# ZackHodari/morgana

Measured on AMD Instinct MI355X. Metric: acoustic frames/sec (fwd+bwd+step), F0Model 600->1, batch 256x1000, higher is better.
Workload: dtype bf16

## Files before the change

### morgana_amd/csrc/optim.hip

```cpp
#include "common.h"
#include "expand_reduce.h"

#include <math.h>

struct mg_adam_out {
    float p, m, v;
};
__device__ __forceinline__ mg_adam_out mg_adam_update(float p, float g, float mi, float vi, float beta1, float beta2, float eps,
                                                       float weight_decay, float step_size, float bc2_sqrt, float grad_scale) {
#pragma clang fp contract(off)
    g = g * grad_scale;
    if (weight_decay != 0.f) g = __fmaf_rn(weight_decay, p, g);
    mi = __fmaf_rn(g - mi, 1.f - beta1, mi);
    vi = __fmaf_rn((1.f - beta2) * g, g, vi * beta2);
    const float denom = sqrtf(vi) / bc2_sqrt + eps;
    p = p - step_size * (mi / denom);
    return mg_adam_out{p, mi, vi};
}

__global__ __launch_bounds__(256) void adam_kernel(float* __restrict__ param, const float* __restrict__ grad,
                                                   float* __restrict__ m, float* __restrict__ v, int64_t n, float beta1,
                                                   float beta2, float eps, float weight_decay, float step_size,
                                                   float bc2_sqrt, float grad_scale) {
    for (int64_t i = (int64_t)blockIdx.x * 256 + threadIdx.x; i < n; i += (int64_t)gridDim.x * 256) {
        const mg_adam_out o = mg_adam_update(param[i], grad[i], m[i], v[i], beta1, beta2, eps, weight_decay, step_size, bc2_sqrt, grad_scale);
        param[i] = o.p;
        m[i] = o.m;
        v[i] = o.v;
    }
}

__global__ __launch_bounds__(256) void adam_dev_kernel(float* __restrict__ param, const float* __restrict__ grad,
                                                       float* __restrict__ m, float* __restrict__ v, int64_t n, float beta1,
                                                       float beta2, float eps, float weight_decay,
                                                       const float* __restrict__ scalars, float grad_scale) {
    const float step_size = scalars[0], bc2_sqrt = scalars[1];
    for (int64_t i = (int64_t)blockIdx.x * 256 + threadIdx.x; i < n; i += (int64_t)gridDim.x * 256) {
        const mg_adam_out o = mg_adam_update(param[i], grad[i], m[i], v[i], beta1, beta2, eps, weight_decay, step_size, bc2_sqrt, grad_scale);
        param[i] = o.p;
        m[i] = o.m;
        v[i] = o.v;
    }
}

__global__ __launch_bounds__(256) void adam_plan_kernel(float* __restrict__ param, float* __restrict__ grad, float* __restrict__ m,
                                                        float* __restrict__ v, int64_t n, float beta1, float beta2, float eps,
                                                        float weight_decay, const float* __restrict__ scalars, float grad_scale,
                                                        mg_adam_plan plan, int wide_chunks) {
    __shared__ float part[16][68];
    if (plan.tail.frames > 0 || plan.tail.n > 0) {
        const mg_adam_tail& t = plan.tail;
        const int64_t by_frames = (t.frames + 2047) / 2048;
        int riders = (int)(by_frames > 1 ? by_frames : 1);
        if (riders > (int)gridDim.x) riders = (int)gridDim.x;
        if ((int)blockIdx.x < riders) {
            const int64_t chunks = (t.n + 15) / 16;
            const ExpandReduceArgs xr{t.table, t.rows, t.frames, t.out, t.partial, t.n_partial, t.slab, t.n, t.stride, t.n_slabs, t.dst,
                                      t.n > 0 ? (t.n - 1) / 16 : chunks};
            mg_expand_reduce_rider<256>(xr, (int)blockIdx.x, riders, reinterpret_cast<unsigned char*>(part));
        }
    }
    const float step_size = scalars[0], bc2_sqrt = scalars[1];
    auto update = [&](int64_t i, float g) {
        if (plan.clear_grad) grad[i] = 0.f;
        const mg_adam_out o = mg_adam_update(param[i], g, m[i], v[i], beta1, beta2, eps, weight_decay, step_size, bc2_sqrt, grad_scale);
        const float w = o.p;
        param[i] = w;
        m[i] = o.m;
        v[i] = o.v;
        for (int k = 0; k < plan.n_shadows; ++k) {
            const mg_adam_shadow sh = plan.shadows[k];
            const int64_t j = i - sh.offset;
            if (j < 0 || j >= (int64_t)sh.rows * sh.cols) continue;
            const unsigned r = (unsigned)j / (unsigned)sh.cols, cc = (unsigned)j - r * (unsigned)sh.cols;
            const uint16_t b = mg_f2bf(w);
            if (sh.dst) sh.dst[(size_t)r * sh.ldd + cc] = b;
            if (sh.dst_t) sh.dst_t[(size_t)cc * sh.ldt + r] = b;
            if (sh.pair) {
                const uint16_t lo = mg_f2bf(w - mg_bf2f(b));
                if (sh.dst) sh.dst[(size_t)r * sh.ldd + (sh.ldd >> 1) + cc] = lo;
                if (sh.dst_t) sh.dst_t[(size_t)cc * sh.ldt + (sh.ldt >> 1) + r] = lo;
            }
        }
    };
    const int e = threadIdx.x & 15, p = threadIdx.x >> 4;
    auto slab_chunk = [&](int64_t base) {
        const int64_t i0 = base + 4 * e;
        f32x4 acc = {0.f, 0.f, 0.f, 0.f};
        bool any = false;
        for (int k = 0; k < plan.n_slab_srcs; ++k) {
            const mg_adam_slab_src src = plan.slabs[k];
            const int64_t j0 = i0 - src.begin;
            if (j0 + 3 < 0 || j0 >= src.count) continue;
            any = true;
            if (j0 >= 0 && j0 + 3 < src.count && ((j0 | src.stride) & 3) == 0 && ((uintptr_t)src.slab & 15) == 0) {
                for (int s = p; s < src.n_slabs; s += 16) acc += *reinterpret_cast<const f32x4*>(src.slab + (size_t)s * src.stride + j0);
            } else {
#pragma unroll
                for (int c = 0; c < 4; ++c) {
                    const int64_t j = j0 + c;
                    if (j < 0 || j >= src.count) continue;
                    float t = 0.f;
                    for (int s = p; s < src.n_slabs; s += 16) t += src.slab[(size_t)s * src.stride + j];
                    acc[c] += t;
                }
            }
        }
        const bool block_any = __syncthreads_or(any ? 1 : 0) != 0;
        if (block_any) {
            *reinterpret_cast<f32x4*>(&part[p][4 * e]) = acc;
            __syncthreads();
        }
        if (threadIdx.x < 64) {
            const int64_t i = base + threadIdx.x;
            if (i < n) {
                float g = grad[i];
                if (block_any) {
#pragma unroll
                    for (int q = 0; q < 16; ++q) g += part[q][threadIdx.x];
                }
                update(i, g);
            }
        }
        if (block_any) __syncthreads();
    };
    if (wide_chunks) {
        const int64_t n_chunks = (n + 255) / 256;
        for (int64_t c = n_chunks - 1 - (int64_t)blockIdx.x; c >= 0; c -= (int64_t)gridDim.x) {
            const int64_t sbase = c * 256;
            bool hit = false;
            for (int k = 0; k < plan.n_slab_srcs; ++k)
                if (sbase < plan.slabs[k].begin + plan.slabs[k].count && sbase + 256 > plan.slabs[k].begin) hit = true;
            if (!hit) {
                const int64_t i = sbase + threadIdx.x;
                if (i < n) update(i, grad[i]);
                continue;
            }
            for (int sub = 3; sub >= 0; --sub)
                if (sbase + 64 * sub < n) slab_chunk(sbase + 64 * sub);
        }
        return;
    }
    const int64_t n_chunks = (n + 63) / 64;
    for (int64_t c = n_chunks - 1 - (int64_t)blockIdx.x; c >= 0; c -= (int64_t)gridDim.x) slab_chunk(c * 64);
}

__global__ __launch_bounds__(256) void ema_kernel(float* __restrict__ shadow, const float* __restrict__ param, int64_t n, float one_minus_decay) {
    for (int64_t i = (int64_t)blockIdx.x * 256 + threadIdx.x; i < n; i += (int64_t)gridDim.x * 256) {
        const float s = shadow[i];
        shadow[i] = s - one_minus_decay * (s - param[i]);
    }
}

__global__ __launch_bounds__(256) void cast_pad_bf16_kernel(const float* __restrict__ src, int lds, uint16_t* __restrict__ dst,
                                                            int ldd, int64_t rows, int cols) {
    const int64_t n = rows * ldd;
    for (int64_t i = (int64_t)blockIdx.x * 256 + threadIdx.x; i < n; i += (int64_t)gridDim.x * 256) {
        const int64_t r = i / ldd;
        const int c = (int)(i - r * ldd);
        dst[i] = c < cols ? mg_f2bf(src[r * lds + c]) : (uint16_t)0;
    }
}

__global__ __launch_bounds__(256) void cast_pad_bf16_x8_kernel(const float* __restrict__ src, int lds, uint16_t* __restrict__ dst,
                                                               int ldd, int64_t rows, int cols) {
    const int chunks = ldd >> 3;
    const int64_t n = rows * chunks;
    for (int64_t i = (int64_t)blockIdx.x * 256 + threadIdx.x; i < n; i += (int64_t)gridDim.x * 256) {
        const int64_t r = i / chunks;
        const int c0 = (int)(i - r * chunks) << 3;
        float v[8];
        const float* sp = src + r * lds + c0;
        if (c0 + 8 <= cols) {
            const f32x4 a = *reinterpret_cast<const f32x4*>(sp), b = *reinterpret_cast<const f32x4*>(sp + 4);
            v[0] = a.x; v[1] = a.y; v[2] = a.z; v[3] = a.w;
            v[4] = b.x; v[5] = b.y; v[6] = b.z; v[7] = b.w;
        } else {
#pragma unroll
            for (int j = 0; j < 8; ++j) v[j] = (c0 + j < cols) ? sp[j] : 0.f;
        }
        bf16x8 o;
#pragma unroll
        for (int j = 0; j < 8; ++j) o[j] = (short)mg_f2bf(v[j]);
        *reinterpret_cast<bf16x8*>(dst + r * ldd + c0) = o;
    }
}

__global__ __launch_bounds__(256) void cast_transpose_bf16_kernel(const float* __restrict__ src, int lds, uint16_t* __restrict__ dst,
                                                                  int ldd, int rows, int cols) {
    __shared__ float tile[32][33];
    const int r0 = blockIdx.y * 32, c0 = blockIdx.x * 32;
    const int tx = threadIdx.x & 31, ty = threadIdx.x >> 5;
    for (int j = ty; j < 32; j += 8) {
        const int r = r0 + j, c = c0 + tx;
        tile[j][tx] = (r < rows && c < cols) ? src[(size_t)r * lds + c] : 0.f;
    }
    __syncthreads();
    for (int j = ty; j < 32; j += 8) {
        const int c = c0 + j, r = r0 + tx;
        if (c < cols && r < ldd) dst[(size_t)c * ldd + r] = r < rows ? mg_f2bf(tile[tx][j]) : (uint16_t)0;
    }
}

__global__ __launch_bounds__(256) void cast_bf16_f32_kernel(const uint16_t* __restrict__ src, int lds, float* __restrict__ dst,
                                                            int ldd, int64_t rows, int cols) {
    const int64_t n = rows * cols;
    for (int64_t i = (int64_t)blockIdx.x * 256 + threadIdx.x; i < n; i += (int64_t)gridDim.x * 256) {
        const int64_t r = i / cols;
        const int c = (int)(i - r * cols);
        dst[r * ldd + c] = mg_bf2f(src[r * lds + c]);
    }
}

__global__ __launch_bounds__(256) void sigmoid_kernel(const float* __restrict__ x, float* __restrict__ y, int64_t n) {
    for (int64_t i = (int64_t)blockIdx.x * 256 + threadIdx.x; i < n; i += (int64_t)gridDim.x * 256) y[i] = mg_sigmoid(x[i]);
}

__global__ __launch_bounds__(256) void sigmoid_grad_kernel(const float* __restrict__ dy, const float* __restrict__ y,
                                                           float* __restrict__ dx, int64_t n) {
    for (int64_t i = (int64_t)blockIdx.x * 256 + threadIdx.x; i < n; i += (int64_t)gridDim.x * 256) {
        const float s = y[i];
        dx[i] = dy[i] * s * (1.f - s);
    }
}

template <int ACT>
__global__ __launch_bounds__(256) void act_kernel(const float* __restrict__ x, float* __restrict__ y, int64_t n) {
    for (int64_t i = (int64_t)blockIdx.x * 256 + threadIdx.x; i < n; i += (int64_t)gridDim.x * 256) {
        const float v = x[i];
        y[i] = ACT == MG_ACT_SIGMOID ? mg_sigmoid(v) : ACT == MG_ACT_TANH ? tanhf(v) : mg_relu(v);
    }
}

template <int EPI>
__global__ __launch_bounds__(256) void act_grad_kernel(const float* __restrict__ dy, const float* __restrict__ y, float* __restrict__ dx,
                                                       int64_t n) {
    for (int64_t i = (int64_t)blockIdx.x * 256 + threadIdx.x; i < n; i += (int64_t)gridDim.x * 256) dx[i] = mg_epi_dact<EPI>(dy[i], y[i]);
}

struct CastBatch {
    int count;
    mg_cast_desc d[MG_CAST_MAX];
};

__global__ __launch_bounds__(256) void cast_params_kernel(CastBatch batch) {
    __shared__ float tile[32][33];
    const mg_cast_desc d = batch.d[blockIdx.y];
    if (d.dst) {
        const int64_t n = (int64_t)d.rows * d.ldd;
        for (int64_t i = (int64_t)blockIdx.x * 256 + threadIdx.x; i < n; i += (int64_t)gridDim.x * 256) {
            const int r = (int)(i / d.ldd), c = (int)(i - (int64_t)r * d.ldd);
            d.dst[i] = c < d.cols ? mg_f2bf(d.src[(size_t)r * d.cols + c]) : (uint16_t)0;
        }
    }
    if (d.dst_t) {
        const int tiles_c = (d.cols + 31) / 32, tiles_r = (d.ldt + 31) / 32;
        const int tx = threadIdx.x & 31, ty = threadIdx.x >> 5;
        for (int t = blockIdx.x; t < tiles_c * tiles_r; t += gridDim.x) {
            const int c0 = (t % tiles_c) * 32, r0 = (t / tiles_c) * 32;
            __syncthreads();
            for (int j = ty; j < 32; j += 8) {
                const int r = r0 + j, c = c0 + tx;
                tile[j][tx] = (r < d.rows && c < d.cols) ? d.src[(size_t)r * d.cols + c] : 0.f;
            }
            __syncthreads();
            for (int j = ty; j < 32; j += 8) {
                const int c = c0 + j, r = r0 + tx;
                if (c < d.cols && r < d.ldt) d.dst_t[(size_t)c * d.ldt + r] = r < d.rows ? mg_f2bf(tile[tx][j]) : (uint16_t)0;
            }
        }
    }
}

struct CopyBatch {
    mg_copy_desc d[MG_COPY_MAX];
};

__global__ __launch_bounds__(256) void copy_many_kernel(CopyBatch batch) {
    const mg_copy_desc d = batch.d[blockIdx.y];
    const unsigned char* src = reinterpret_cast<const unsigned char*>(d.src);
    unsigned char* dst = reinterpret_cast<unsigned char*>(d.dst);
    const int64_t stride = (int64_t)gridDim.x * 256;
    if ((((uintptr_t)src | (uintptr_t)dst) & 15) == 0) {
        const int64_t n16 = d.bytes >> 4;
        typedef unsigned int cm_u32x4 __attribute__((ext_vector_type(4)));
        for (int64_t i = (int64_t)blockIdx.x * 256 + threadIdx.x; i < n16; i += stride)
            reinterpret_cast<cm_u32x4*>(dst)[i] = reinterpret_cast<const cm_u32x4*>(src)[i];
        for (int64_t i = (n16 << 4) + (int64_t)blockIdx.x * 256 + threadIdx.x; i < d.bytes; i += stride) dst[i] = src[i];
    } else {
        for (int64_t i = (int64_t)blockIdx.x * 256 + threadIdx.x; i < d.bytes; i += stride) dst[i] = src[i];
    }
}

static int flat_grid(int64_t n) {
    int64_t blocks = mg_ceil_div(n, 256 * 4);
    if (blocks > 4096) blocks = 4096;
    return (int)(blocks < 1 ? 1 : blocks);
}

extern "C" {

int mg_adam_step_f32(float* param, const float* grad, float* exp_avg, float* exp_avg_sq, int64_t n, float lr, float beta1,
                     float beta2, float eps, float weight_decay, int64_t step, float grad_scale, void* stream) {
    MG_CHECK_ARG(param && grad && exp_avg && exp_avg_sq && n >= 0 && step >= 1, "mg_adam_step_f32: bad arguments (n=%lld step=%lld)",
                 (long long)n, (long long)step);
    if (n == 0) return MG_OK;
    const double bc1 = 1.0 - pow((double)beta1, (double)step);
    const double bc2 = 1.0 - pow((double)beta2, (double)step);
    const float step_size = (float)((double)lr / bc1);
    const float bc2_sqrt = (float)sqrt(bc2);
    hipLaunchKernelGGL(adam_kernel, dim3(flat_grid(n)), dim3(256), 0, (hipStream_t)stream, param, grad, exp_avg, exp_avg_sq, n,
                       beta1, beta2, eps, weight_decay, step_size, bc2_sqrt, grad_scale);
    MG_CHECK_LAUNCH("mg_adam_step_f32");
    return MG_OK;
}

__global__ void store_pair_kernel(float* __restrict__ dst, float a, float b) {
    dst[0] = a;
    dst[1] = b;
}

int mg_store_pair_f32(float* dst, float a, float b, void* stream) {
    MG_CHECK_ARG(dst, "mg_store_pair_f32: null destination");
    hipLaunchKernelGGL(store_pair_kernel, dim3(1), dim3(1), 0, (hipStream_t)stream, dst, a, b);
    MG_CHECK_LAUNCH("mg_store_pair_f32");
    return MG_OK;
}

struct StorePairs {
    float v[2 * MG_STORE_PAIRS_MAX];
};
__global__ void store_pairs_kernel(float* __restrict__ dst, StorePairs values, int n) {
    if ((int)threadIdx.x < 2 * n) dst[threadIdx.x] = values.v[threadIdx.x];
}

int mg_store_pairs_f32(float* dst, const float* values, int n_pairs, void* stream) {
    MG_CHECK_ARG(dst && values && n_pairs >= 1 && n_pairs <= MG_STORE_PAIRS_MAX, "mg_store_pairs_f32: bad arguments (n_pairs=%d, at most %d)", n_pairs,
                 MG_STORE_PAIRS_MAX);
    StorePairs sp;
    for (int i = 0; i < 2 * n_pairs; ++i) sp.v[i] = values[i];
    for (int i = 2 * n_pairs; i < 2 * MG_STORE_PAIRS_MAX; ++i) sp.v[i] = 0.f;
    hipLaunchKernelGGL(store_pairs_kernel, dim3(1), dim3(64), 0, (hipStream_t)stream, dst, sp, n_pairs);
    MG_CHECK_LAUNCH("mg_store_pairs_f32");
    return MG_OK;
}

void mg_adam_scalars(float lr, float beta1, float beta2, int64_t step, float* out2) {
    const double bc1 = 1.0 - pow((double)beta1, (double)step);
    const double bc2 = 1.0 - pow((double)beta2, (double)step);
    out2[0] = (float)((double)lr / bc1);
    out2[1] = (float)sqrt(bc2);
}

int mg_adam_step_dev_f32(float* param, const float* grad, float* exp_avg, float* exp_avg_sq, int64_t n, float beta1, float beta2,
                         float eps, float weight_decay, const float* scalars, float grad_scale, void* stream) {
    MG_CHECK_ARG(param && grad && exp_avg && exp_avg_sq && scalars && n >= 0, "mg_adam_step_dev_f32: bad arguments (n=%lld)", (long long)n);
    if (n == 0) return MG_OK;
    hipLaunchKernelGGL(adam_dev_kernel, dim3(flat_grid(n)), dim3(256), 0, (hipStream_t)stream, param, grad, exp_avg, exp_avg_sq, n,
                       beta1, beta2, eps, weight_decay, scalars, grad_scale);
    MG_CHECK_LAUNCH("mg_adam_step_dev_f32");
    return MG_OK;
}

int mg_adam_step_plan_f32(float* param, float* grad, float* exp_avg, float* exp_avg_sq, int64_t n, float beta1, float beta2, float eps,
                          float weight_decay, const float* scalars, float grad_scale, const mg_adam_plan* plan, void* stream) {
    MG_CHECK_ARG(param && grad && exp_avg && exp_avg_sq && scalars && plan && n >= 0, "mg_adam_step_plan_f32: bad arguments (n=%lld)", (long long)n);
    MG_CHECK_ARG(plan->n_slab_srcs >= 0 && plan->n_slab_srcs <= MG_ADAM_MAX_SLABS && plan->n_shadows >= 0 && plan->n_shadows <= MG_ADAM_MAX_SHADOWS,
                 "mg_adam_step_plan_f32: %d slab sources / %d shadows exceed %d / %d", plan->n_slab_srcs, plan->n_shadows, MG_ADAM_MAX_SLABS,
                 MG_ADAM_MAX_SHADOWS);
    for (int k = 0; k < plan->n_slab_srcs; ++k) {
        const mg_adam_slab_src& src = plan->slabs[k];
        MG_CHECK_ARG(src.slab && src.begin >= 0 && src.count > 0 && src.begin + src.count <= n && src.n_slabs >= 1 && src.stride >= src.count,
                     "mg_adam_step_plan_f32: slab source %d (begin %lld count %lld of %lld, %d slabs, stride %lld)", k, (long long)src.begin,
                     (long long)src.count, (long long)n, src.n_slabs, (long long)src.stride);
    }
    for (int k = 0; k < plan->n_shadows; ++k) {
        const mg_adam_shadow& sh = plan->shadows[k];
        MG_CHECK_ARG(sh.offset >= 0 && sh.rows > 0 && sh.cols > 0 && (int64_t)sh.rows * sh.cols < 2147483647LL &&
                         sh.offset + (int64_t)sh.rows * sh.cols <= n && (sh.dst || sh.dst_t),
                     "mg_adam_step_plan_f32: shadow %d does not lie inside the flat buffer", k);
        MG_CHECK_ARG((!sh.dst || sh.ldd >= sh.cols) && (!sh.dst_t || sh.ldt >= sh.rows), "mg_adam_step_plan_f32: shadow %d: ldd %d / ldt %d too small", k,
                     sh.ldd, sh.ldt);
        MG_CHECK_ARG(!sh.pair || ((!sh.dst || (sh.ldd % 2 == 0 && sh.ldd / 2 >= sh.cols)) && (!sh.dst_t || (sh.ldt % 2 == 0 && sh.ldt / 2 >= sh.rows))),
                     "mg_adam_step_plan_f32: shadow %d: pair planes need even ldd %d / ldt %d with half of it covering the matrix", k, sh.ldd, sh.ldt);
    }
    {
        const mg_adam_tail& t = plan->tail;
        MG_CHECK_ARG(t.frames >= 0 && t.n >= 0 && (t.frames == 0 || (t.table && t.rows && t.out)) &&
                         (t.n == 0 || (t.slab && t.dst && t.stride >= t.n && t.n_slabs >= 1 && (t.n_partial == 0 || t.partial))),
                     "mg_adam_step_plan_f32: bad deferred tail (frames %lld, n %lld)", (long long)t.frames, (long long)t.n);
        MG_CHECK_ARG((t.frames == 0 && t.n == 0) || n > 0, "mg_adam_step_plan_f32: a deferred tail needs a launch (n = 0)");
    }
    if (n == 0) return MG_OK;
    int64_t covered = 0;
    for (int k = 0; k < plan->n_slab_srcs; ++k) covered += plan->slabs[k].count;
    const int wide = 2 * covered < n ? 1 : 0;
    hipLaunchKernelGGL(adam_plan_kernel, dim3((unsigned)mg_ceil_div(n, wide ? 256 : 64)), dim3(256), 0, (hipStream_t)stream, param, grad, exp_avg,
                       exp_avg_sq, n, beta1, beta2, eps, weight_decay, scalars, grad_scale, *plan, wide);
    MG_CHECK_LAUNCH("mg_adam_step_plan_f32");
    return MG_OK;
}

int mg_ema_update_f32(float* shadow, const float* param, int64_t n, float decay, void* stream) {
    MG_CHECK_ARG(shadow && param && n >= 0, "mg_ema_update_f32: bad arguments");
    if (n == 0) return MG_OK;
    hipLaunchKernelGGL(ema_kernel, dim3(flat_grid(n)), dim3(256), 0, (hipStream_t)stream, shadow, param, n, 1.0f - decay);
    MG_CHECK_LAUNCH("mg_ema_update_f32");
    return MG_OK;
}

int mg_cast_pad_bf16(const float* src, int lds, uint16_t* dst, int ldd, int64_t rows, int cols, void* stream) {
    MG_CHECK_ARG(src && dst && rows >= 0 && cols > 0 && lds >= cols && ldd >= cols, "mg_cast_pad_bf16: bad arguments (rows=%lld cols=%d lds=%d ldd=%d)",
                 (long long)rows, cols, lds, ldd);
    if (rows == 0) return MG_OK;
    if (lds % 4 == 0 && ldd % 8 == 0 && (((uintptr_t)src | (uintptr_t)dst) % 16) == 0)
        hipLaunchKernelGGL(cast_pad_bf16_x8_kernel, dim3(flat_grid(rows * (ldd / 8))), dim3(256), 0, (hipStream_t)stream, src, lds, dst, ldd, rows, cols);
    else
        hipLaunchKernelGGL(cast_pad_bf16_kernel, dim3(flat_grid(rows * ldd)), dim3(256), 0, (hipStream_t)stream, src, lds, dst, ldd, rows, cols);
    MG_CHECK_LAUNCH("mg_cast_pad_bf16");
    return MG_OK;
}

int mg_cast_transpose_bf16(const float* src, int lds, uint16_t* dst, int ldd, int rows, int cols, void* stream) {
    MG_CHECK_ARG(src && dst && rows > 0 && cols > 0 && lds >= cols && ldd >= rows, "mg_cast_transpose_bf16: bad arguments (rows=%d cols=%d lds=%d ldd=%d)",
                 rows, cols, lds, ldd);
    dim3 grid((unsigned)mg_ceil_div(cols, 32), (unsigned)mg_ceil_div(ldd, 32));
    hipLaunchKernelGGL(cast_transpose_bf16_kernel, grid, dim3(256), 0, (hipStream_t)stream, src, lds, dst, ldd, rows, cols);
    MG_CHECK_LAUNCH("mg_cast_transpose_bf16");
    return MG_OK;
}

int mg_cast_params_bf16(const mg_cast_desc* descs, int count, void* stream) {
    MG_CHECK_ARG(descs && count > 0 && count <= MG_CAST_MAX, "mg_cast_params_bf16: count %d not in 1..%d", count, MG_CAST_MAX);
    CastBatch batch;
    batch.count = count;
    for (int i = 0; i < count; ++i) {
        const mg_cast_desc& d = descs[i];
        MG_CHECK_ARG(d.src && d.rows > 0 && d.cols > 0 && (d.dst || d.dst_t), "mg_cast_params_bf16: bad descriptor %d", i);
        MG_CHECK_ARG(!d.dst || d.ldd >= d.cols, "mg_cast_params_bf16: descriptor %d: ldd %d < cols %d", i, d.ldd, d.cols);
        MG_CHECK_ARG(!d.dst_t || d.ldt >= d.rows, "mg_cast_params_bf16: descriptor %d: ldt %d < rows %d", i, d.ldt, d.rows);
        batch.d[i] = d;
    }
    hipLaunchKernelGGL(cast_params_kernel, dim3(256, count), dim3(256), 0, (hipStream_t)stream, batch);
    MG_CHECK_LAUNCH("mg_cast_params_bf16");
    return MG_OK;
}

int mg_copy_many(const mg_copy_desc* descs, int count, void* stream) {
    MG_CHECK_ARG(descs && count > 0 && count <= MG_COPY_MAX, "mg_copy_many: count %d not in 1..%d", count, MG_COPY_MAX);
    CopyBatch batch;
    int64_t most = 0;
    for (int i = 0; i < count; ++i) {
        MG_CHECK_ARG(descs[i].bytes >= 0 && (descs[i].bytes == 0 || (descs[i].src && descs[i].dst)), "mg_copy_many: bad descriptor %d", i);
        batch.d[i] = descs[i];
        if (descs[i].bytes > most) most = descs[i].bytes;
    }
    if (most == 0) return MG_OK;
    int64_t blocks = mg_ceil_div(most, 256 * 16 * 4);
    if (blocks > 2048) blocks = 2048;
    if (blocks < 1) blocks = 1;
    hipLaunchKernelGGL(copy_many_kernel, dim3((unsigned)blocks, count), dim3(256), 0, (hipStream_t)stream, batch);
    MG_CHECK_LAUNCH("mg_copy_many");
    return MG_OK;
}

int mg_cast_bf16_f32(const uint16_t* src, int lds, float* dst, int ldd, int64_t rows, int cols, void* stream) {
    MG_CHECK_ARG(src && dst && rows >= 0 && cols > 0 && lds >= cols && ldd >= cols, "mg_cast_bf16_f32: bad arguments");
    if (rows == 0) return MG_OK;
    hipLaunchKernelGGL(cast_bf16_f32_kernel, dim3(flat_grid(rows * cols)), dim3(256), 0, (hipStream_t)stream, src, lds, dst, ldd, rows, cols);
    MG_CHECK_LAUNCH("mg_cast_bf16_f32");
    return MG_OK;
}

int mg_sigmoid_f32(const float* x, float* y, int64_t n, void* stream) {
    MG_CHECK_ARG(x && y && n >= 0, "mg_sigmoid_f32: bad arguments");
    if (n == 0) return MG_OK;
    hipLaunchKernelGGL(sigmoid_kernel, dim3(flat_grid(n)), dim3(256), 0, (hipStream_t)stream, x, y, n);
    MG_CHECK_LAUNCH("mg_sigmoid_f32");
    return MG_OK;
}

int mg_sigmoid_grad_f32(const float* dy, const float* y, float* dx, int64_t n, void* stream) {
    MG_CHECK_ARG(dy && y && dx && n >= 0, "mg_sigmoid_grad_f32: bad arguments");
    if (n == 0) return MG_OK;
    hipLaunchKernelGGL(sigmoid_grad_kernel, dim3(flat_grid(n)), dim3(256), 0, (hipStream_t)stream, dy, y, dx, n);
    MG_CHECK_LAUNCH("mg_sigmoid_grad_f32");
    return MG_OK;
}

int mg_act_f32(const float* x, float* y, int64_t n, int act, void* stream) {
    MG_CHECK_ARG(x && y && n >= 0, "mg_act_f32: bad arguments");
    MG_CHECK_ARG(act == MG_ACT_SIGMOID || act == MG_ACT_TANH || act == MG_ACT_RELU, "mg_act_f32: unknown activation %d", act);
    if (n == 0) return MG_OK;
    if (act == MG_ACT_SIGMOID) hipLaunchKernelGGL(act_kernel<MG_ACT_SIGMOID>, dim3(flat_grid(n)), dim3(256), 0, (hipStream_t)stream, x, y, n);
    else if (act == MG_ACT_TANH) hipLaunchKernelGGL(act_kernel<MG_ACT_TANH>, dim3(flat_grid(n)), dim3(256), 0, (hipStream_t)stream, x, y, n);
    else hipLaunchKernelGGL(act_kernel<MG_ACT_RELU>, dim3(flat_grid(n)), dim3(256), 0, (hipStream_t)stream, x, y, n);
    MG_CHECK_LAUNCH("mg_act_f32");
    return MG_OK;
}

int mg_act_grad_f32(const float* dy, const float* y, float* dx, int64_t n, int act, void* stream) {
    MG_CHECK_ARG(dy && y && dx && n >= 0, "mg_act_grad_f32: bad arguments");
    MG_CHECK_ARG(act == MG_ACT_SIGMOID || act == MG_ACT_TANH || act == MG_ACT_RELU, "mg_act_grad_f32: unknown activation %d", act);
    if (n == 0) return MG_OK;
#define ACT_GRAD(EPI_) hipLaunchKernelGGL(act_grad_kernel<EPI_>, dim3(flat_grid(n)), dim3(256), 0, (hipStream_t)stream, dy, y, dx, n)
    MG_SWITCH_GRAD_EPI(mg_epi_grad(act), ACT_GRAD);
#undef ACT_GRAD
    MG_CHECK_LAUNCH("mg_act_grad_f32");
    return MG_OK;
}

}
```

### morgana_amd/csrc/slab_reduce.h

```cpp
#pragma once

#include "common.h"

static __global__ __launch_bounds__(256) void mg_slab_reduce_kernel(const float* __restrict__ slab, int64_t n, int64_t stride,
                                                                    int S, float* __restrict__ dst, int accumulate) {
    __shared__ float part[16][17];
    const int e = threadIdx.x & 15, p = threadIdx.x >> 4;
    for (int64_t base = (int64_t)blockIdx.x * 16; base < n; base += (int64_t)gridDim.x * 16) {
        const int64_t i = base + e;
        float v = 0.f;
        if (i < n) {
#pragma unroll 4
            for (int s = p; s < S; s += 16) v += slab[(size_t)s * stride + i];
        }
        part[p][e] = v;
        __syncthreads();
        if (p == 0 && i < n) {
            float t = accumulate ? dst[i] : 0.f;
#pragma unroll
            for (int q = 0; q < 16; ++q) t += part[q][e];
            dst[i] = t;
        }
        __syncthreads();
    }
}

static __global__ __launch_bounds__(256) void mg_slab_reduce4_kernel(const float* __restrict__ slab, int64_t n, int64_t stride,
                                                                     int S, float* __restrict__ dst, int accumulate) {
    __shared__ f32x4 part[16][17];
    const int e = threadIdx.x & 15, p = threadIdx.x >> 4;
    for (int64_t base = (int64_t)blockIdx.x * 64; base < n; base += (int64_t)gridDim.x * 64) {
        const int64_t i = base + 4 * e;
        f32x4 v = {0.f, 0.f, 0.f, 0.f};
        if (i < n) {
#pragma unroll 4
            for (int s = p; s < S; s += 16) v += *reinterpret_cast<const f32x4*>(slab + (size_t)s * stride + i);
        }
        part[p][e] = v;
        __syncthreads();
        if (p == 0 && i < n) {
            f32x4 t = {0.f, 0.f, 0.f, 0.f};
            if (accumulate) t = *reinterpret_cast<const f32x4*>(dst + i);
#pragma unroll
            for (int q = 0; q < 16; ++q) t += part[q][e];
            *reinterpret_cast<f32x4*>(dst + i) = t;
        }
        __syncthreads();
    }
}

static inline void mg_launch_slab_reduce(const float* slab, int64_t n, int64_t stride, int S, float* dst, int accumulate,
                                         hipStream_t st) {
#ifdef MG_EXPERIMENTS
    if (g_mg_tuning[MG_TUNE_SKIP_REDUCE]) return;
#endif
    if (n % 4 == 0 && stride % 4 == 0 && n >= 4096 && (((uintptr_t)slab | (uintptr_t)dst) % 16) == 0) {
        int64_t blocks4 = mg_ceil_div(n, 64);
        if (blocks4 > 32768) blocks4 = 32768;
        hipLaunchKernelGGL(mg_slab_reduce4_kernel, dim3((unsigned)blocks4), dim3(256), 0, st, slab, n, stride, S, dst, accumulate);
        return;
    }
    int64_t blocks = mg_ceil_div(n, 16);
    if (blocks > 32768) blocks = 32768;
    if (blocks < 1) blocks = 1;
    hipLaunchKernelGGL(mg_slab_reduce_kernel, dim3((unsigned)blocks), dim3(256), 0, st, slab, n, stride, S, dst, accumulate);
}
```

Baseline: 2.499 billion.

## Restructure fused Adam kernel to per-wave 256-element chunks with register slab sums

The fused Adam plan kernel is rewritten so that each wave owns a 256-element chunk, with lanes processing four elements through vectorised loads and stores. The cross-thread reduction through shared memory and its block barriers is replaced by per-lane register accumulation of slab partial sums, with loads batched 16 or 32 at a time. The grid is capped at a fixed block count with launch bounds asking for two blocks per CU, and bf16 shadow writes are packed four at a time. The risks are high register pressure from the 16 f32x4 accumulators, and much less parallelism across the slab dimension, since each lane now serially sums all slabs.

```diff
diff --git a/morgana_amd/csrc/optim.hip b/morgana_amd/csrc/optim.hip
--- a/morgana_amd/csrc/optim.hip
+++ b/morgana_amd/csrc/optim.hip
@@ -1,5 +1,6 @@
 #include "common.h"
 #include "expand_reduce.h"
+#include "slab_reduce.h"
 
 #include <math.h>
 
@@ -43,12 +44,23 @@
     }
 }
 
-__global__ __launch_bounds__(256) void adam_plan_kernel(float* __restrict__ param, float* __restrict__ grad, float* __restrict__ m,
-                                                        float* __restrict__ v, int64_t n, float beta1, float beta2, float eps,
-                                                        float weight_decay, const float* __restrict__ scalars, float grad_scale,
-                                                        mg_adam_plan plan, int wide_chunks) {
-    __shared__ float part[16][68];
+__device__ __noinline__ void mg_adam_edge_sums(const float* __restrict__ slab, int64_t stride, int S, int64_t j0, int64_t count, float* t) {
+    for (int e = 0; e < 4; ++e) {
+        const int64_t j = j0 + e;
+        if (j < 0 || j >= count) continue;
+        for (int s = 0; s < S; ++s) t[(s & 15) * 4 + e] += slab[(int64_t)s * stride + j];
+    }
+}
+
+#ifndef MG_ADAM_PLAN_BLOCKS
+#define MG_ADAM_PLAN_BLOCKS 1024
+#endif
+__global__ __launch_bounds__(256, 2) void adam_plan_kernel(float* __restrict__ param, float* __restrict__ grad, float* __restrict__ m,
+                                                           float* __restrict__ v, int64_t n, float beta1, float beta2, float eps,
+                                                           float weight_decay, const float* __restrict__ scalars, float grad_scale,
+                                                           mg_adam_plan plan) {
     if (plan.tail.frames > 0 || plan.tail.n > 0) {
+        __shared__ float rider_scratch[16 * 17 + 256];
         const mg_adam_tail& t = plan.tail;
         const int64_t by_frames = (t.frames + 2047) / 2048;
         int riders = (int)(by_frames > 1 ? by_frames : 1);
@@ -57,92 +69,144 @@
             const int64_t chunks = (t.n + 15) / 16;
             const ExpandReduceArgs xr{t.table, t.rows, t.frames, t.out, t.partial, t.n_partial, t.slab, t.n, t.stride, t.n_slabs, t.dst,
                                       t.n > 0 ? (t.n - 1) / 16 : chunks};
-            mg_expand_reduce_rider<256>(xr, (int)blockIdx.x, riders, reinterpret_cast<unsigned char*>(part));
+            mg_expand_reduce_rider<256>(xr, (int)blockIdx.x, riders, reinterpret_cast<unsigned char*>(rider_scratch));
         }
     }
     const float step_size = scalars[0], bc2_sqrt = scalars[1];
-    auto update = [&](int64_t i, float g) {
-        if (plan.clear_grad) grad[i] = 0.f;
-        const mg_adam_out o = mg_adam_update(param[i], g, m[i], v[i], beta1, beta2, eps, weight_decay, step_size, bc2_sqrt, grad_scale);
-        const float w = o.p;
-        param[i] = w;
-        m[i] = o.m;
-        v[i] = o.v;
+    auto put = [&](const mg_adam_shadow& sh, unsigned r, unsigned cc, float w, bool hi_done) {
+        const uint16_t b = mg_f2bf(w);
+        if (sh.dst && !hi_done) sh.dst[(size_t)r * sh.ldd + cc] = b;
+        if (sh.dst_t) sh.dst_t[(size_t)cc * sh.ldt + r] = b;
+        if (sh.pair) {
+            const uint16_t lo = mg_f2bf(w - mg_bf2f(b));
+            if (sh.dst) sh.dst[(size_t)r * sh.ldd + (sh.ldd >> 1) + cc] = lo;
+            if (sh.dst_t) sh.dst_t[(size_t)cc * sh.ldt + (sh.ldt >> 1) + r] = lo;
+        }
+    };
+    const int lane = threadIdx.x & 63;
+    const unsigned voff = 16u * (unsigned)lane;
+    const int wave = __builtin_amdgcn_readfirstlane((int)(threadIdx.x >> 6));
+    const bool state_vec = ((((uintptr_t)param | (uintptr_t)grad | (uintptr_t)m | (uintptr_t)v) & 15) == 0);
+    const int64_t n_chunks = (n + 255) / 256;
+    for (int64_t c = n_chunks - 1 - ((int64_t)wave * gridDim.x + blockIdx.x); c >= 0; c -= 4 * (int64_t)gridDim.x) {
+        const int64_t base = c * 256, i0 = base + 4 * lane;
+        const bool whole = state_vec && base + 256 <= n;
+        f32x4 g4 = {0.f, 0.f, 0.f, 0.f}, p4 = g4, m4 = g4, v4 = g4;
+        if (whole) {
+            g4 = *reinterpret_cast<const f32x4*>(grad + i0);
+            p4 = *reinterpret_cast<const f32x4*>(param + i0);
+            m4 = *reinterpret_cast<const f32x4*>(m + i0);
+            v4 = *reinterpret_cast<const f32x4*>(v + i0);
+        } else {
+#pragma unroll
+            for (int e = 0; e < 4; ++e)
+                if (i0 + e < n) {
+                    g4[e] = grad[i0 + e];
+                    p4[e] = param[i0 + e];
+                    m4[e] = m[i0 + e];
+                    v4[e] = v[i0 + e];
+                }
+        }
+        f32x4 t[16];
+#pragma unroll
+        for (int q = 0; q < 16; ++q) t[q] = f32x4{0.f, 0.f, 0.f, 0.f};
+        unsigned covered = 0;
+#pragma unroll 1
+        for (int k = 0; k < plan.n_slab_srcs; ++k) {
+            const mg_adam_slab_src src = plan.slabs[k];
+            const int64_t jb = base - src.begin;
+            if (jb + 256 <= 0 || jb >= src.count) continue;
+            const int64_t j0 = jb + 4 * lane;
+#pragma unroll
+            for (int e = 0; e < 4; ++e)
+                if (j0 + e >= 0 && j0 + e < src.count) covered |= 1u << e;
+            if (((jb | src.stride) & 3) == 0 && ((uintptr_t)src.slab & 15) == 0) {
+                const bool inside = j0 >= 0 && j0 < src.count;
+                const float* sp = src.slab + jb;
+                mg_slab_partition_sums(src.n_slabs, t, [&](int s) {
+                    f32x4 x = {0.f, 0.f, 0.f, 0.f};
+                    if (inside) x = *reinterpret_cast<const f32x4*>(reinterpret_cast<const char*>(sp + (size_t)s * src.stride) + voff);
+                    return x;
+                });
+            } else {
+                float tm[64];
+#pragma unroll
+                for (int q = 0; q < 16; ++q)
+#pragma unroll
+                    for (int e = 0; e < 4; ++e) tm[4 * q + e] = t[q][e];
+                mg_adam_edge_sums(src.slab, src.stride, src.n_slabs, j0, src.count, tm);
+#pragma unroll
+                for (int q = 0; q < 16; ++q)
+#pragma unroll
+                    for (int e = 0; e < 4; ++e) t[q][e] = tm[4 * q + e];
+            }
+        }
+        if (covered) {
+            f32x4 gs = g4;
+#pragma unroll
+            for (int q = 0; q < 16; ++q) gs += t[q];
+#pragma unroll
+            for (int e = 0; e < 4; ++e)
+                if (covered >> e & 1) g4[e] = gs[e];
+        }
+        f32x4 w4;
+#pragma unroll
+        for (int e = 0; e < 4; ++e) {
+            const mg_adam_out o = mg_adam_update(p4[e], g4[e], m4[e], v4[e], beta1, beta2, eps, weight_decay, step_size, bc2_sqrt, grad_scale);
+            w4[e] = o.p;
+            m4[e] = o.m;
+            v4[e] = o.v;
+        }
+        if (whole) {
+            if (plan.clear_grad) *reinterpret_cast<f32x4*>(grad + i0) = f32x4{0.f, 0.f, 0.f, 0.f};
+            *reinterpret_cast<f32x4*>(param + i0) = w4;
+            *reinterpret_cast<f32x4*>(m + i0) = m4;
+            *reinterpret_cast<f32x4*>(v + i0) = v4;
+        } else {
+#pragma unroll
+            for (int e = 0; e < 4; ++e)
+                if (i0 + e < n) {
+                    if (plan.clear_grad) grad[i0 + e] = 0.f;
+                    param[i0 + e] = w4[e];
+                    m[i0 + e] = m4[e];
+                    v[i0 + e] = v4[e];
+                }
+        }
+#pragma unroll 1
         for (int k = 0; k < plan.n_shadows; ++k) {
             const mg_adam_shadow sh = plan.shadows[k];
-            const int64_t j = i - sh.offset;
-            if (j < 0 || j >= (int64_t)sh.rows * sh.cols) continue;
-            const unsigned r = (unsigned)j / (unsigned)sh.cols, cc = (unsigned)j - r * (unsigned)sh.cols;
-            const uint16_t b = mg_f2bf(w);
-            if (sh.dst) sh.dst[(size_t)r * sh.ldd + cc] = b;
-            if (sh.dst_t) sh.dst_t[(size_t)cc * sh.ldt + r] = b;
-            if (sh.pair) {
-                const uint16_t lo = mg_f2bf(w - mg_bf2f(b));
-                if (sh.dst) sh.dst[(size_t)r * sh.ldd + (sh.ldd >> 1) + cc] = lo;
-                if (sh.dst_t) sh.dst_t[(size_t)cc * sh.ldt + (sh.ldt >> 1) + r] = lo;
-            }
-        }
-    };
-    const int e = threadIdx.x & 15, p = threadIdx.x >> 4;
-    auto slab_chunk = [&](int64_t base) {
-        const int64_t i0 = base + 4 * e;
-        f32x4 acc = {0.f, 0.f, 0.f, 0.f};
-        bool any = false;
-        for (int k = 0; k < plan.n_slab_srcs; ++k) {
-            const mg_adam_slab_src src = plan.slabs[k];
-            const int64_t j0 = i0 - src.begin;
-            if (j0 + 3 < 0 || j0 >= src.count) continue;
-            any = true;
-            if (j0 >= 0 && j0 + 3 < src.count && ((j0 | src.stride) & 3) == 0 && ((uintptr_t)src.slab & 15) == 0) {
-                for (int s = p; s < src.n_slabs; s += 16) acc += *reinterpret_cast<const f32x4*>(src.slab + (size_t)s * src.stride + j0);
+            const int64_t rc = (int64_t)sh.rows * sh.cols, jb = base - sh.offset;
+            if (jb + 256 <= 0 || jb >= rc) continue;
+            const int64_t j0 = jb + 4 * lane;
+            if (j0 + 3 < 0 || j0 >= rc) continue;
+            const unsigned jf = (unsigned)(j0 > 0 ? j0 : 0), cols = (unsigned)sh.cols;
+            unsigned r = jf / cols, cc = jf - r * cols;
+            if (j0 >= 0 && j0 + 3 < rc && cc + 3 < cols) {
+                uint16_t* d = sh.dst ? sh.dst + (size_t)r * sh.ldd + cc : nullptr;
+                const bool packed = d && ((uintptr_t)d & 7) == 0;
+                if (packed) {
+                    bf16x4 b;
+#pragma unroll
+                    for (int e = 0; e < 4; ++e) b[e] = (short)mg_f2bf(w4[e]);
+                    *reinterpret_cast<bf16x4*>(d) = b;
+                }
+                if (!packed || sh.dst_t || sh.pair) {
+#pragma unroll
+                    for (int e = 0; e < 4; ++e) put(sh, r, cc + e, w4[e], packed);
+                }
             } else {
 #pragma unroll
-                for (int c = 0; c < 4; ++c) {
-                    const int64_t j = j0 + c;
-                    if (j < 0 || j >= src.count) continue;
-                    float t = 0.f;
-                    for (int s = p; s < src.n_slabs; s += 16) t += src.slab[(size_t)s * src.stride + j];
-                    acc[c] += t;
+                for (int e = 0; e < 4; ++e) {
+                    if (j0 + e < 0 || j0 + e >= rc) continue;
+                    put(sh, r, cc, w4[e], false);
+                    if (++cc == cols) {
+                        cc = 0;
+                        ++r;
+                    }
                 }
             }
         }
-        const bool block_any = __syncthreads_or(any ? 1 : 0) != 0;
-        if (block_any) {
-            *reinterpret_cast<f32x4*>(&part[p][4 * e]) = acc;
-            __syncthreads();
-        }
-        if (threadIdx.x < 64) {
-            const int64_t i = base + threadIdx.x;
-            if (i < n) {
-                float g = grad[i];
-                if (block_any) {
-#pragma unroll
-                    for (int q = 0; q < 16; ++q) g += part[q][threadIdx.x];
-                }
-                update(i, g);
-            }
-        }
-        if (block_any) __syncthreads();
-    };
-    if (wide_chunks) {
-        const int64_t n_chunks = (n + 255) / 256;
-        for (int64_t c = n_chunks - 1 - (int64_t)blockIdx.x; c >= 0; c -= (int64_t)gridDim.x) {
-            const int64_t sbase = c * 256;
-            bool hit = false;
-            for (int k = 0; k < plan.n_slab_srcs; ++k)
-                if (sbase < plan.slabs[k].begin + plan.slabs[k].count && sbase + 256 > plan.slabs[k].begin) hit = true;
-            if (!hit) {
-                const int64_t i = sbase + threadIdx.x;
-                if (i < n) update(i, grad[i]);
-                continue;
-            }
-            for (int sub = 3; sub >= 0; --sub)
-                if (sbase + 64 * sub < n) slab_chunk(sbase + 64 * sub);
-        }
-        return;
-    }
-    const int64_t n_chunks = (n + 63) / 64;
-    for (int64_t c = n_chunks - 1 - (int64_t)blockIdx.x; c >= 0; c -= (int64_t)gridDim.x) slab_chunk(c * 64);
+    }
 }
 
 __global__ __launch_bounds__(256) void ema_kernel(float* __restrict__ shadow, const float* __restrict__ param, int64_t n, float one_minus_decay) {
@@ -392,11 +456,10 @@
         MG_CHECK_ARG((t.frames == 0 && t.n == 0) || n > 0, "mg_adam_step_plan_f32: a deferred tail needs a launch (n = 0)");
     }
     if (n == 0) return MG_OK;
-    int64_t covered = 0;
-    for (int k = 0; k < plan->n_slab_srcs; ++k) covered += plan->slabs[k].count;
-    const int wide = 2 * covered < n ? 1 : 0;
-    hipLaunchKernelGGL(adam_plan_kernel, dim3((unsigned)mg_ceil_div(n, wide ? 256 : 64)), dim3(256), 0, (hipStream_t)stream, param, grad, exp_avg,
-                       exp_avg_sq, n, beta1, beta2, eps, weight_decay, scalars, grad_scale, *plan, wide);
+    int64_t blocks = mg_ceil_div(n, 256);
+    if (blocks > MG_ADAM_PLAN_BLOCKS) blocks = MG_ADAM_PLAN_BLOCKS;
+    hipLaunchKernelGGL(adam_plan_kernel, dim3((unsigned)blocks), dim3(256), 0, (hipStream_t)stream, param, grad, exp_avg, exp_avg_sq, n, beta1,
+                       beta2, eps, weight_decay, scalars, grad_scale, *plan);
     MG_CHECK_LAUNCH("mg_adam_step_plan_f32");
     return MG_OK;
 }
diff --git a/morgana_amd/csrc/slab_reduce.h b/morgana_amd/csrc/slab_reduce.h
--- a/morgana_amd/csrc/slab_reduce.h
+++ b/morgana_amd/csrc/slab_reduce.h
@@ -1,6 +1,42 @@
 #pragma once
 
 #include "common.h"
+
+#ifndef MG_SLAB_ROUND
+#define MG_SLAB_ROUND 32
+#endif
+template <class Load>
+__device__ __forceinline__ void mg_slab_partition_sums(int S, f32x4 (&t)[16], Load load) {
+    int s0 = 0;
+#if MG_SLAB_ROUND == 32
+    for (; s0 + 32 <= S; s0 += 32) {
+        f32x4 a[16], b[16];
+#pragma unroll
+        for (int q = 0; q < 16; ++q) a[q] = load(s0 + q);
+#pragma unroll
+        for (int q = 0; q < 16; ++q) b[q] = load(s0 + 16 + q);
+#pragma unroll
+        for (int q = 0; q < 16; ++q) t[q] += a[q];
+#pragma unroll
+        for (int q = 0; q < 16; ++q) t[q] += b[q];
+    }
+#endif
+    for (; s0 + 16 <= S; s0 += 16) {
+        f32x4 a[16];
+#pragma unroll
+        for (int q = 0; q < 16; ++q) a[q] = load(s0 + q);
+#pragma unroll
+        for (int q = 0; q < 16; ++q) t[q] += a[q];
+    }
+    if (s0 == S) return;
+    f32x4 d[15];
+#pragma unroll
+    for (int q = 0; q < 15; ++q)
+        if (s0 + q < S) d[q] = load(s0 + q);
+#pragma unroll
+    for (int q = 0; q < 15; ++q)
+        if (s0 + q < S) t[q] += d[q];
+}
 
 static __global__ __launch_bounds__(256) void mg_slab_reduce_kernel(const float* __restrict__ slab, int64_t n, int64_t stride,
                                                                     int S, float* __restrict__ dst, int accumulate) {
```

New measurement: 2.409 billion. 0.964x the previous value.
